# Hiroto1201/Open3D-ML

Measured on AMD Instinct MI355X. Metric: Mpoints/s neighbor-search + sparse-conv fwd; RandLA-Net frames/s, higher is better.
Workload: dtype f32; 1 GPU; C1 fixed_radius_search: layers.FixedRadiusSearch forward (hash build + search) over 64 scenes/GPU x 65,536 U[0,1)^3 pts, r=0.05, L2, int32 idx; scenes_per_gpu=64, parallelism=scene-dp1

## Files before the change

### open3d-ml_amd/csrc/nns_hash.hip

```cpp
#include <algorithm>
#include <cstdlib>

#include "primitives.hpp"
#include "spatial_hash.hpp"

namespace o3dml {

__global__ void __launch_bounds__(256) hash_points_kernel(const float* __restrict__ points, int64_t n, float inv,
                                                          int n_batch, const int64_t* __restrict__ prs,
                                                          const uint32_t* __restrict__ hts,
                                                          uint32_t* __restrict__ bins) {
    __shared__ int64_t s_rs[kLdsSplits];
    __shared__ uint32_t s_tab[kLdsSplits][3];
    const int64_t* rsp = stage_splits(s_rs, prs, n_batch);
    const bool tab = n_batch <= kLdsSplits;
    if (tab) {
        for (int b = threadIdx.x; b < n_batch; b += blockDim.x) {
            const uint32_t first = hts[b], tsize = hts[b + 1] - first;
            s_tab[b][0] = first;
            s_tab[b][1] = tsize;
            s_tab[b][2] = pow64_mod(tsize);
        }
        __syncthreads();
    }
// ... 72 lines not shown
    }
    __syncthreads();
}

__global__ void __launch_bounds__(256) hash_plan_kernel(const int64_t* __restrict__ prs, int nb,
                                                        const uint32_t* __restrict__ hts,
                                                        int64_t* __restrict__ chunk_start,
                                                        int64_t* __restrict__ hist_off, int chunk) {
    hash_plan_block(prs, nb, hts, chunk, chunk_start, hist_off);
}

constexpr int kPlanLds = 512;

__device__ __forceinline__ bool hash_chunk_of(const int64_t* __restrict__ chunk_start, int nb, int& b, int64_t& c) {
    const int64_t w = blockIdx.x;
    if (w >= chunk_start[nb]) return false;
    int lo = 0, hi = nb - 1;
    while (lo < hi) {
        const int mid = (lo + hi + 1) >> 1;
        if (chunk_start[mid] <= w) lo = mid; else hi = mid - 1;
    }
    b = lo;
    c = w - chunk_start[lo];
    return true;
}

template <bool PLAN>
__global__ void __launch_bounds__(256) hash_chunk_hist_kernel(const float* __restrict__ points, float inv, int nb,
                                                              const int64_t* __restrict__ prs,
                                                              const uint32_t* __restrict__ hts,
                                                              int64_t* __restrict__ chunk_start,
                                                              int64_t* __restrict__ hist_off,
                                                              uint32_t* __restrict__ bins, uint32_t* __restrict__ hist,
                                                              int chunk) {
    extern __shared__ uint32_t h[];
    __shared__ int64_t s_plan[PLAN ? 2 * kPlanLds : 1];
    const int64_t* cs = chunk_start;
    const int64_t* ho = hist_off;
    if constexpr (PLAN) {
        hash_plan_block(prs, nb, hts, chunk, s_plan, s_plan + kPlanLds);
        if (blockIdx.x == 0)
            for (int i = threadIdx.x; i <= nb; i += 256) {
                chunk_start[i] = s_plan[i];
                hist_off[i] = s_plan[kPlanLds + i];
            }
        cs = s_plan;
        ho = s_plan + kPlanLds;
    }
    int b;
    int64_t c;
    if (!hash_chunk_of(cs, nb, b, c)) return;
    const int64_t* hist_off_ = ho;
    const uint32_t tsize = hts[b + 1] - hts[b];
    const uint32_t k64 = pow64_mod(tsize);
    for (uint32_t i = threadIdx.x; i < tsize; i += 256) h[i] = 0;
    __syncthreads();
    const int64_t p0 = prs[b] + c * chunk, p1 = min(prs[b + 1], p0 + chunk);
    constexpr int U = 8;
    for (int64_t i0 = p0 + threadIdx.x; i0 < p1; i0 += 256 * U) {
        float px[U], py[U], pz[U];
#pragma unroll
        for (int u = 0; u < U; ++u) {
            const int64_t i = i0 + 256 * u;
            const int64_t j = i < p1 ? i : p0;
            px[u] = points[3 * j];
            py[u] = points[3 * j + 1];
            pz[u] = points[3 * j + 2];
        }
#pragma unroll
        for (int u = 0; u < U; ++u) {
            const int64_t i = i0 + 256 * u;
            if (i < p1) {
                const uint32_t bin = point_bin_k(px[u], py[u], pz[u], inv, tsize, k64);
                bins[i] = bin;
                atomicAdd(&h[bin], 1u);
            }
        }
    }
    __syncthreads();
    uint32_t* out = hist + hist_off_[b] + c * tsize;
    for (uint32_t i = threadIdx.x; i < tsize; i += 256) out[i] = h[i];
}

constexpr int kColBins = 64;
__global__ void __launch_bounds__(256) hash_hist_colscan_kernel(int nslices, const uint32_t* __restrict__ hts,
                                                                const int64_t* __restrict__ chunk_start,
                                                                const int64_t* __restrict__ hist_off,
                                                                uint32_t* __restrict__ hist,
                                                                uint32_t* __restrict__ bin_tot) {
    __shared__ uint32_t qsum[4][kColBins];
    const int b = blockIdx.x / nslices, s = blockIdx.x % nslices;
    const int q = wave_id(), lane = lane_id();
    const uint32_t first = hts[b], tsize = hts[b + 1] - first;
    const uint32_t bin = static_cast<uint32_t>(s * kColBins + lane);
    if (static_cast<uint32_t>(s * kColBins) >= tsize) return;
    const bool valid = bin < tsize;
    const int64_t nchunks = chunk_start[b + 1] - chunk_start[b];
    const int64_t c0 = nchunks * q / 4, c1 = nchunks * (q + 1) / 4;
    uint32_t* H = hist + hist_off[b] + bin;
    uint32_t sum = 0;
    if (valid) {
        int64_t cc = c0;
        for (; cc + 8 <= c1; cc += 8) {
            uint32_t v[8];
#pragma unroll
            for (int u = 0; u < 8; ++u) v[u] = H[(cc + u) * tsize];
            sum += ((v[0] + v[1]) + (v[2] + v[3])) + ((v[4] + v[5]) + (v[6] + v[7]));
        }
        for (; cc < c1; ++cc) sum += H[cc * tsize];
    }
    qsum[q][lane] = sum;
    __syncthreads();
    uint32_t run = 0;
    for (int k = 0; k < q; ++k) run += qsum[k][lane];
    if (valid) {
        if (q == 3) bin_tot[first + bin] = run + sum;
        int64_t cc = c0;
        for (; cc + 8 <= c1; cc += 8) {
            uint32_t v[8];
#pragma unroll
            for (int u = 0; u < 8; ++u) v[u] = H[(cc + u) * tsize];
#pragma unroll
            for (int u = 0; u < 8; ++u) {
                H[(cc + u) * tsize] = run;
                run += v[u];
            }
        }
        for (; cc < c1; ++cc) {
            const uint32_t v = H[cc * tsize];
            H[cc * tsize] = run;
            run += v;
        }
    }
}

template <int CHUNK, int NWV = kHashWaves>
__global__ void __launch_bounds__(NWV * 64) hash_chunk_scatter_kernel(int nb, const int64_t* __restrict__ prs,
                                                                 const uint32_t* __restrict__ hts,
                                                                 const int64_t* __restrict__ chunk_start,
                                                                 const int64_t* __restrict__ hist_off,
                                                                 const uint32_t* __restrict__ bins,
                                                                 const uint32_t* __restrict__ hist,
                                                                 const uint32_t* __restrict__ bin_tot,
                                                                 uint32_t* __restrict__ cell_splits,
                                                                 uint32_t* __restrict__ hti, int max_bins) {
    constexpr int kRows = CHUNK / 64 / NWV;
    extern __shared__ uint32_t wc_all[];
    __shared__ uint32_t wsum[NWV];
    int b;
    int64_t c;
    if (!hash_chunk_of(chunk_start, nb, b, c)) return;
    const int t = threadIdx.x, w = wave_id(), lane = lane_id();
    const uint32_t first = hts[b], tsize = hts[b + 1] - first;
    const int64_t item0 = prs[b], item_end = prs[b + 1];
    const uint32_t* base = hist + hist_off[b] + c * tsize;
    uint32_t* wc = wc_all + w * max_bins;
    uint32_t* bstart = wc_all + NWV * max_bins;
    for (uint32_t i = t; i < tsize; i += NWV * 64)
#pragma unroll
        for (int ww = 0; ww < NWV; ++ww) wc_all[ww * max_bins + i] = 0;
    {
        uint32_t carry = 0;
        for (uint32_t b0 = 0; b0 < tsize; b0 += NWV * 64) {
            const uint32_t i = b0 + t;
            const uint32_t v = i < tsize ? bin_tot[first + i] : 0u;
            const uint32_t inc = wave_inclusive_scan(v);
            if (lane == 63) wsum[w] = inc;
            __syncthreads();
            uint32_t st = carry + inc - v, all = 0;
#pragma unroll
            for (int ww = 0; ww < NWV; ++ww) {
                st += ww < w ? wsum[ww] : 0u;
                all += wsum[ww];
            }
            if (i < tsize) {
                bstart[i] = st;
                if (c == 0) cell_splits[first + i] = static_cast<uint32_t>(item0 + st);
            }
            carry += all;
            __syncthreads();
        }
        if (c == 0 && b == nb - 1 && t == 0) cell_splits[first + tsize] = static_cast<uint32_t>(prs[nb]);
    }
    __syncthreads();
    const int64_t p0 = item0 + c * CHUNK;
    const int64_t pend = min(item_end, p0 + CHUNK);
    const int nbits = tsize > 1 ? 32 - __builtin_clz(tsize - 1) : 0;
    const uint64_t lt = lanemask_lt();
    uint32_t dig[kRows], loff[kRows];
#pragma unroll
    for (int r = 0; r < kRows; ++r) {
        const int64_t i = p0 + (static_cast<int64_t>(w) * kRows + r) * 64 + lane;
        dig[r] = bins[i < pend ? i : p0];
    }
#pragma unroll
    for (int r = 0; r < kRows; ++r) {
        const int64_t i = p0 + (static_cast<int64_t>(w) * kRows + r) * 64 + lane;
        const bool valid = i < pend;
        const uint32_t d = valid ? dig[r] : 0u;
        dig[r] = d;
        uint64_t peers = __builtin_amdgcn_ballot_w64(valid);
        for (int bit = 0; bit < nbits; ++bit) {
            const bool on = (d >> bit) & 1u;
            const uint64_t m = __builtin_amdgcn_ballot_w64(on);
            peers &= on ? m : ~m;
        }
        const uint32_t rank = __popcll(peers & lt);
        const uint32_t before = valid ? wc[d] : 0u;
        loff[r] = before + rank;
        if (valid && rank == 0) wc[d] = before + static_cast<uint32_t>(__popcll(peers));
    }
    __syncthreads();
    for (uint32_t i = t; i < tsize; i += NWV * 64) {
        uint32_t a = bstart[i] + base[i];
#pragma unroll
        for (int ww = 0; ww < NWV; ++ww) {
            const uint32_t cw = wc_all[ww * max_bins + i];
            wc_all[ww * max_bins + i] = a;
            a += cw;
        }
    }
    __syncthreads();
#pragma unroll
    for (int r = 0; r < kRows; ++r) {
        const int64_t i = p0 + (static_cast<int64_t>(w) * kRows + r) * 64 + lane;
        if (i < pend) hti[item0 + wc[dig[r]] + loff[r]] = static_cast<uint32_t>(i);
    }
}

}

using namespace o3dml;

O3DML_API int64_t o3dml_hash_table_splits(int64_t n_batch, const int64_t* points_row_splits_host,
                                          double hash_table_size_factor, int64_t max_hash_table_size,
                                          uint32_t* hash_table_splits_host) {
    hash_table_splits_host[0] = 0;
    for (int64_t b = 0; b < n_batch; ++b) {
        const int64_t nb = points_row_splits_host[b + 1] - points_row_splits_host[b];
        int64_t t = static_cast<int64_t>(hash_table_size_factor * static_cast<double>(nb));
        if (t < 1) t = 1;
        if (t > max_hash_table_size) t = max_hash_table_size;
        hash_table_splits_host[b + 1] = hash_table_splits_host[b] + static_cast<uint32_t>(t);
    }
    return hash_table_splits_host[n_batch];
}

O3DML_API size_t o3dml_build_spatial_hash_table_workspace_size(int64_t n_points, int64_t total_bins) {
    const size_t radix = ws_bytes<uint32_t>(n_points) * 2 + prim::radix_sort_workspace_bytes<uint32_t>(n_points);
    const int64_t nb_ub = total_bins;
    const int64_t hist_ub = 4 * n_points + total_bins;
    const size_t small = ws_bytes<uint32_t>(n_points) + ws_bytes<uint32_t>(hist_ub) +
                         ws_bytes<uint32_t>(total_bins) + 2 * ws_bytes<int64_t>(nb_ub + 1);
    return std::max(radix, small);
}

O3DML_API int o3dml_build_spatial_hash_table(const float* points, int64_t n_points, float radius, int64_t n_batch,
                                             const int64_t* points_row_splits, const uint32_t* hash_table_splits,
                                             const uint32_t* hash_table_splits_host, int64_t total_bins,
                                             uint32_t* hash_table_index, uint32_t* hash_table_cell_splits,
                                             void* workspace, size_t workspace_bytes, void* stream) {
    O3DML_GUARD_BEGIN
    O3DML_REQUIRE(radius > 0.f, "radius must be > 0");
    O3DML_REQUIRE(n_batch >= 1, "need at least one batch item");
    O3DML_REQUIRE(total_bins >= n_batch && total_bins < (int64_t(1) << 32), "invalid hash table size %lld",
                  (long long)total_bins);
    hipStream_t st = as_stream(stream);
    Workspace ws(workspace, workspace_bytes);
    const float inv = 1.0f / (2.0f * radius);
    bool small = hash_table_splits_host != nullptr && n_points > 0;
    uint32_t max_bins = 1;
    for (int64_t b = 0; small && b < n_batch; ++b) {
        const uint32_t tb = hash_table_splits_host[b + 1] - hash_table_splits_host[b];
        max_bins = std::max(max_bins, tb);
        small = tb <= static_cast<uint32_t>(kSmallTable);
    }
    if (small) {
        uint32_t* bins = ws.take<uint32_t>(n_points);
        static const int forced = [] {
            const char* e = std::getenv("O3DML_HASH_CHUNK");
            const int v = e ? std::atoi(e) : 0;
            return (v == 1024 || v == 2048 || v == 4096) ? v : 0;
        }();
        const int chunk = forced ? forced : (ceil_div(n_points, kHashChunk) < 512 ? kHashChunkSmall : kHashChunk);
        uint32_t* hist = ws.take<uint32_t>((kHashChunk / chunk) * n_points + total_bins);
        uint32_t* bin_tot = ws.take<uint32_t>(total_bins);
        int64_t* chunk_start = ws.take<int64_t>(n_batch + 1);
        int64_t* hist_off = ws.take<int64_t>(n_batch + 1);
        const unsigned grid = static_cast<unsigned>(ceil_div(n_points, chunk) + n_batch);
        if (n_batch < kPlanLds) {
            hash_chunk_hist_kernel<true><<<grid, 256, sizeof(uint32_t) * max_bins, st>>>(
                    points, inv, (int)n_batch, points_row_splits, hash_table_splits, chunk_start, hist_off, bins,
                    hist, chunk);
        } else {
            hash_plan_kernel<<<1, 256, 0, st>>>(points_row_splits, (int)n_batch, hash_table_splits, chunk_start,
                                                hist_off, chunk);
            O3DML_LAUNCH_CHECK();
            hash_chunk_hist_kernel<false><<<grid, 256, sizeof(uint32_t) * max_bins, st>>>(
                    points, inv, (int)n_batch, points_row_splits, hash_table_splits, chunk_start, hist_off, bins,
                    hist, chunk);
        }
        O3DML_LAUNCH_CHECK();
        const int nslices = static_cast<int>(ceil_div(max_bins, kColBins));
        hash_hist_colscan_kernel<<<static_cast<unsigned>(n_batch * nslices), 256, 0, st>>>(
                nslices, hash_table_splits, chunk_start, hist_off, hist, bin_tot);
        O3DML_LAUNCH_CHECK();
        const size_t lds = sizeof(uint32_t) * (kHashWaves + 1) * max_bins;
        static const int hw = [] {
            const char* e = std::getenv("O3DML_HASH_WAVES");
            return e ? std::atoi(e) : 4;
        }();
        const size_t lds8 = sizeof(uint32_t) * 9 * max_bins;
        if (chunk == kHashChunkSmall)
            hash_chunk_scatter_kernel<kHashChunkSmall><<<grid, 256, lds, st>>>(
                    (int)n_batch, points_row_splits, hash_table_splits, chunk_start, hist_off, bins, hist, bin_tot,
                    hash_table_cell_splits, hash_table_index, static_cast<int>(max_bins));
        else if (chunk == 2048)
            hash_chunk_scatter_kernel<2048><<<grid, 256, lds, st>>>(
                    (int)n_batch, points_row_splits, hash_table_splits, chunk_start, hist_off, bins, hist, bin_tot,
                    hash_table_cell_splits, hash_table_index, static_cast<int>(max_bins));
        else if (hw == 8 && lds8 <= 65536)
            hash_chunk_scatter_kernel<kHashChunk, 8><<<grid, 512, lds8, st>>>(
                    (int)n_batch, points_row_splits, hash_table_splits, chunk_start, hist_off, bins, hist, bin_tot,
                    hash_table_cell_splits, hash_table_index, static_cast<int>(max_bins));
        else
            hash_chunk_scatter_kernel<kHashChunk><<<grid, 256, lds, st>>>(
                    (int)n_batch, points_row_splits, hash_table_splits, chunk_start, hist_off, bins, hist, bin_tot,
                    hash_table_cell_splits, hash_table_index, static_cast<int>(max_bins));
        O3DML_LAUNCH_CHECK();
        return 0;
    }
    uint32_t* bins = ws.take<uint32_t>(n_points);
    uint32_t* skeys = ws.take<uint32_t>(n_points);
    if (n_points > 0) {
        hash_points_kernel<<<stream_grid(n_points, 256), 256, 0, st>>>(points, n_points, inv, (int)n_batch,
                                                                      points_row_splits, hash_table_splits, bins);
        O3DML_LAUNCH_CHECK();
        prim::radix_sort_pairs<uint32_t>(bins, nullptr, skeys, hash_table_index, n_points,
                                         prim::bits_needed(static_cast<uint64_t>(total_bins - 1)), ws, st);
    }
    bin_boundaries_kernel<<<stream_grid(n_points > 0 ? n_points : total_bins + 1, 256), 256, 0, st>>>(
            skeys, n_points, total_bins, hash_table_cell_splits);
    O3DML_LAUNCH_CHECK();
    O3DML_GUARD_END
}
```

### open3d-ml_amd/csrc/common.hpp

```cpp
#pragma once

#include <hip/hip_runtime.h>

#include <cstdint>
#include <cstdio>
#include <cstring>
#include <string>

#include "../../include/o3dml_amd.h"

#define O3DML_API extern "C" __attribute__((visibility("default")))

namespace o3dml {

void set_error(const char* fmt, ...);
const char* last_error();

struct Error {
    int code;
};

#define O3DML_CHECK_HIP(expr)                                                   \
    do {                                                                        \
        hipError_t _e = (expr);                                                 \
// ... 91 lines not shown
    return (static_cast<size_t>(count < 0 ? 0 : count) * sizeof(T) + 255) & ~size_t(255);
}

__device__ __forceinline__ float sum_slabs(const float* __restrict__ part, int nsplit, int64_t total, int64_t e) {
    float v = 0.f;
    int s = 0;
    for (; s + 16 <= nsplit; s += 16) {
        float t[16];
#pragma unroll
        for (int j = 0; j < 16; ++j) t[j] = part[(s + j) * total + e];
#pragma unroll
        for (int j = 0; j < 16; ++j) v += t[j];
    }
    for (; s < nsplit; ++s) v += part[s * total + e];
    return v;
}

__device__ __forceinline__ int lane_id() { return threadIdx.x & 63; }
__device__ __forceinline__ int wave_id() { return threadIdx.x >> 6; }

__device__ __forceinline__ uint64_t lanemask_lt() {
    const int l = lane_id();
    return l == 0 ? 0ull : (~0ull >> (64 - l));
}

template <class T>
__device__ __forceinline__ T wave_inclusive_scan(T v) {
#pragma unroll
    for (int d = 1; d < 64; d <<= 1) {
        T t = __shfl_up(v, d, 64);
        if (lane_id() >= d) v += t;
    }
    return v;
}

template <class T>
__device__ __forceinline__ T wave_sum(T v) {
#pragma unroll
    for (int d = 32; d >= 1; d >>= 1) v += __shfl_xor(v, d, 64);
    return v;
}

template <class T>
__device__ __forceinline__ T wave_max(T v) {
#pragma unroll
    for (int d = 32; d >= 1; d >>= 1) {
        const T o = __shfl_xor(v, d, 64);
        v = o > v ? o : v;
    }
    return v;
}

__device__ __forceinline__ float dist_l2(float px, float py, float pz, float qx, float qy, float qz) {
    const float dx = px - qx, dy = py - qy, dz = pz - qz;
    return __builtin_fmaf(dz, dz, __builtin_fmaf(dy, dy, dx * dx));
}

enum Metric { kL1 = 0, kL2 = 1, kLinf = 2 };

template <int METRIC>
__device__ __forceinline__ float dist_metric(float px, float py, float pz, float qx, float qy, float qz) {
    if constexpr (METRIC == kL2) {
        return dist_l2(px, py, pz, qx, qy, qz);
    } else {
        const float ax = fabsf(px - qx), ay = fabsf(py - qy), az = fabsf(pz - qz);
        if constexpr (METRIC == kL1) {
            return (ax + ay) + az;
        } else {
            const float m = ax > ay ? ax : ay;
            return m > az ? m : az;
        }
    }
}

__device__ __forceinline__ int batch_of(int64_t i, const int64_t* __restrict__ splits, int n_batch) {
    int lo = 0, hi = n_batch - 1;
    while (lo < hi) {
        int mid = (lo + hi + 1) >> 1;
        if (splits[mid] <= i) lo = mid; else hi = mid - 1;
    }
    return lo;
}

template <int LANE>
__device__ __forceinline__ int write_lane(int v, int x) {
    asm volatile("v_writelane_b32 %0, %1, %2" : "+v"(v) : "s"(x), "i"(LANE));
    return v;
}

constexpr int kBufferFlags = 0x00020000;

constexpr int kLdsSplits = 1024;
__device__ __forceinline__ const int64_t* stage_splits(int64_t* lds, const int64_t* __restrict__ splits,
                                                       int n_batch) {
    if (n_batch + 1 > kLdsSplits) return splits;
    for (int i = threadIdx.x; i <= n_batch; i += blockDim.x) lds[i] = splits[i];
    __syncthreads();
    return lds;
}

__device__ __forceinline__ int64_t xcd_block() {
    const int64_t g = gridDim.x, b = blockIdx.x;
    return (g & 7) ? b : (b & 7) * (g >> 3) + (b >> 3);
}

inline unsigned xcd_grid(int64_t n, int block) {
    int64_t g = ceil_div(n, 4 * static_cast<int64_t>(block));
    g = ((g + 7) / 8) * 8;
    if (g < 8) g = 8;
    if (g > 2048) g = 2048;
    return static_cast<unsigned>(g);
}

}
```

### open3d-ml_amd/csrc/nns_frs.hip

```cpp
#include <algorithm>
#include <cstdlib>
#include <mutex>

#include "primitives.hpp"
#include "spatial_hash.hpp"

namespace o3dml {

__global__ void __launch_bounds__(256) gather_sorted_points_kernel(const float* __restrict__ points,
                                                                   const uint32_t* __restrict__ index, int64_t n,
                                                                   float4* __restrict__ out, int sentinel,
                                                                   int64_t* __restrict__ zero_a, int n_zero_a,
                                                                   int64_t* __restrict__ zero_b) {
    const int64_t per = ceil_div(n, static_cast<int64_t>(gridDim.x));
    const int64_t blk = xcd_block();
    const int64_t e = min(n, (blk + 1) * per);
    constexpr int U = 4;
    for (int64_t j0 = blk * per + threadIdx.x; j0 < e; j0 += U * static_cast<int64_t>(blockDim.x)) {
        uint32_t id[U];
#pragma unroll
        for (int u = 0; u < U; ++u) {
            const int64_t j = j0 + u * static_cast<int64_t>(blockDim.x);
            id[u] = j < e ? index[j] : 0u;
        }
// ... 80 lines not shown
O3DML_DPP_STEP(dmax_rm, "v_max_f32", "row_mirror")
#undef O3DML_DPP_STEP
template <bool MAX>
__device__ __forceinline__ float row_ext_f(float v) {
#if O3DML_FRS_DPPMIN
    if constexpr (MAX) return dmax_rm(dmax_hm(dmax_q2(dmax_q1(v))));
    return dmin_rm(dmin_hm(dmin_q2(dmin_q1(v))));
#else
    auto op = [](float a, float b) { return MAX ? fmaxf(a, b) : fminf(a, b); };
    v = op(v, dpp_f<0xB1>(v));
    v = op(v, dpp_f<0x4E>(v));
    v = op(v, dpp_f<0x141>(v));
    v = op(v, dpp_f<0x140>(v));
    return v;
#endif
}
__device__ __forceinline__ float rdlane_f(float v, int l) {
    return __int_as_float(__builtin_amdgcn_readlane(__float_as_int(v), l));
}
__device__ __forceinline__ float wave_min_f(float v) {
    v = row_ext_f<false>(v);
    return fminf(fminf(rdlane_f(v, 0), rdlane_f(v, 16)), fminf(rdlane_f(v, 32), rdlane_f(v, 48)));
}
__device__ __forceinline__ float wave_max_f(float v) {
    v = row_ext_f<true>(v);
    return fmaxf(fmaxf(rdlane_f(v, 0), rdlane_f(v, 16)), fmaxf(rdlane_f(v, 32), rdlane_f(v, 48)));
}
__device__ __forceinline__ float row0_min_f(float v) { return rdlane_f(row_ext_f<false>(v), 0); }
__device__ __forceinline__ float row0_max_f(float v) { return rdlane_f(row_ext_f<true>(v), 0); }

template <int METRIC>
__device__ __forceinline__ float box_dist(const float4& p, float lx, float ly, float lz, float hx, float hy,
                                          float hz) {
    const float gx = p.x - __builtin_amdgcn_fmed3f(p.x, lx, hx);
    const float gy = p.y - __builtin_amdgcn_fmed3f(p.y, ly, hy);
    const float gz = p.z - __builtin_amdgcn_fmed3f(p.z, lz, hz);
    if constexpr (METRIC == kL2) {
        return __builtin_fmaf(gz, gz, __builtin_fmaf(gy, gy, gx * gx));
    } else if constexpr (METRIC == kL1) {
        return (fabsf(gx) + fabsf(gy)) + fabsf(gz);
    } else {
        const float ax = fabsf(gx), ay = fabsf(gy), az = fabsf(gz);
        const float m = ax > ay ? ax : ay;
        return m > az ? m : az;
    }
}

template <int METRIC>
__device__ __forceinline__ float box_box_dist(float alx, float aly, float alz, float ahx, float ahy, float ahz,
                                              float blx, float bly, float blz, float bhx, float bhy, float bhz) {
    const float gx = fmaxf(fmaxf(alx - bhx, blx - ahx), 0.f);
    const float gy = fmaxf(fmaxf(aly - bhy, bly - ahy), 0.f);
    const float gz = fmaxf(fmaxf(alz - bhz, blz - ahz), 0.f);
    if constexpr (METRIC == kL2) {
        return __builtin_fmaf(gz, gz, __builtin_fmaf(gy, gy, gx * gx));
    } else if constexpr (METRIC == kL1) {
        return (gx + gy) + gz;
    } else {
        const float m = gx > gy ? gx : gy;
        return m > gz ? m : gz;
    }
}

__device__ __forceinline__ int keep_slot(uint64_t km) {
    return static_cast<int>(__builtin_amdgcn_mbcnt_hi(static_cast<uint32_t>(km >> 32),
                                                      __builtin_amdgcn_mbcnt_lo(static_cast<uint32_t>(km), 0u)));
}

__device__ __forceinline__ uint32_t mbcnt64(uint64_t m) {
    return __builtin_amdgcn_mbcnt_hi(static_cast<uint32_t>(m >> 32),
                                     __builtin_amdgcn_mbcnt_lo(static_cast<uint32_t>(m), 0u));
}

__device__ __forceinline__ uint32_t bcnt_add(uint32_t x, uint32_t acc) {
    uint32_t r;
    asm("v_bcnt_u32_b32 %0, %1, %2" : "=v"(r) : "v"(x), "v"(acc));
    return r;
}

__device__ __forceinline__ uint32_t rdlane(int v, uint32_t lane) {
    return static_cast<uint32_t>(__builtin_amdgcn_readlane(v, static_cast<int>(lane)));
}

template <int K>
__device__ __forceinline__ int bin_lanes(int v, const uint32_t* lb) {
    if constexpr (K < 9) return bin_lanes<K + 1>(write_lane<K>(v, static_cast<int>(lb[K])), lb);
    return v;
}

#ifndef O3DML_FRS_NUM_SGPR
#define O3DML_FRS_NUM_SGPR 80
#endif
#ifndef O3DML_FRS_WAVES
#define O3DML_FRS_WAVES 8
#endif
#ifndef O3DML_FRS_ABS16
#define O3DML_FRS_ABS16 1
#endif
#define O3DML_FRS_ATTR \
    __attribute__((amdgpu_num_sgpr(O3DML_FRS_NUM_SGPR), amdgpu_waves_per_eu(DIST ? 1 : O3DML_FRS_WAVES, 8)))
template <int METRIC, bool IGNORE, bool DIST, int MODE, class TIdx, bool REL16>
__global__ void __launch_bounds__(64) O3DML_FRS_ATTR
frs_group_kernel(const float4* __restrict__ pts, uint32_t n_pts, const uint32_t* __restrict__ cs,
                 const float4* __restrict__ qpts, const uint32_t* __restrict__ qsel,
                 const uint32_t* __restrict__ qkeys, int bshift, int64_t m_host, const int64_t* __restrict__ m_dev,
                 float r, float inv, float thr, int nb, const int64_t* __restrict__ qrs,
                 const uint32_t* __restrict__ hts, const int64_t* __restrict__ prs,
                 uint32_t* __restrict__ counts, uint32_t* __restrict__ tidx,
                 float* __restrict__ tdist, uint32_t* __restrict__ over, int64_t* __restrict__ n_over,
                 const int64_t* __restrict__ rs, TIdx* __restrict__ out_idx, float* __restrict__ out_dist,
                 const int64_t* __restrict__ total, int64_t cap, const uint32_t* __restrict__ dir,
                 int64_t dir_cap, int qlog, int64_t dense_w) {
    __shared__ float4 cand[kCandCap];
    __shared__ float4 qsh[64];
    __shared__ int64_t qrow[MODE == 0 ? 1 : 64];
    const int lane = threadIdx.x;
    const float inf = __builtin_huge_valf();
    const float4 far = make_float4(inf, inf, inf, 0.f);
    const int64_t m = MODE == 1 && cap >= 0 && *total > cap ? 0 : (m_dev ? *m_dev : m_host);
    const int64_t nchunks = MODE == 0 ? (m + (1 << qlog) - 1) >> qlog : m;
    const bool pts_rsrc_ok = n_pts < 0x07FFFFFEu;
    const bool sub = dir != nullptr && static_cast<int64_t>(hts[nb]) <= dir_cap;
    const __amdgpu_buffer_rsrc_t rows_rsrc = __builtin_amdgcn_make_buffer_rsrc(
            tidx, static_cast<short>(0), REL16 ? static_cast<int>(m * 2 * kRowCap) : 0, kBufferFlags);
    const __amdgpu_buffer_rsrc_t pts_rsrc = __builtin_amdgcn_make_buffer_rsrc(
            const_cast<float4*>(pts), static_cast<short>(0), static_cast<int>((2u * n_pts + 1u) * 16u), kBufferFlags);
    const int64_t per = (nchunks + 7) >> 3;
    const bool xcd_map = static_cast<int64_t>(gridDim.x) == 8 * per;
    int64_t chunk = xcd_map ? static_cast<int64_t>(blockIdx.x & 7) * per + (blockIdx.x >> 3) : blockIdx.x;
    for (; chunk < nchunks; chunk = xcd_map ? nchunks : chunk + gridDim.x) {
        const int64_t t = MODE == 0 ? (chunk << qlog) + lane : chunk;
        const bool valid = t < m && (MODE == 0 ? lane < (1 << qlog) : lane == 0);
        float4 q4 = far;
        QueryBins qb;
#pragma unroll
        for (int k = 0; k < 9; ++k) qb.b[k] = 0xffffffffu;
        int64_t row = 0;
        uint32_t pbase = 0;
        if (valid) {
            if constexpr (MODE == 0) {
                if (qsel) {
                    const uint32_t qs = qsel[t];
                    if (qpts) {
                        const float* qp = reinterpret_cast<const float*>(qpts) + 3 * static_cast<int64_t>(qs);
                        q4 = make_float4(qp[0], qp[1], qp[2], __uint_as_float(qs));
                    } else {
                        q4 = pts[qs];
                    }
                } else {
                    q4 = qpts[t];
                }
            } else {
                const uint32_t id = over[t];
                const float* qp = reinterpret_cast<const float*>(qpts) + 3 * static_cast<int64_t>(id);
                q4 = make_float4(qp[0], qp[1], qp[2], __uint_as_float(id));
            }
            const uint32_t qid = __float_as_uint(q4.w);
            const int b = qkeys ? (bshift >= 32 ? 0 : static_cast<int>(qkeys[t] >> bshift)) : batch_of(qid, qrs, nb);
            if constexpr (REL16) pbase = static_cast<uint32_t>(prs[b]);
            const uint32_t first = hts[b], tsize = hts[b + 1] - first;
            qb = query_bins(q4.x, q4.y, q4.z, r, inv, first, tsize);
            if constexpr (MODE == 1) row = dense_w > 0 ? static_cast<int64_t>(qid) * dense_w : rs[qid];
        }
        uint64_t todo = __builtin_amdgcn_ballot_w64(valid);
        while (todo) {
            const int leader = __builtin_ctzll(todo);
            uint32_t lb[9];
            bool same = valid;
#pragma unroll
            for (int k = 0; k < 9; ++k) {
                lb[k] = rdlane(static_cast<int>(qb.b[k]), leader);
                same = same && qb.b[k] == lb[k];
            }
            const uint64_t gm = __builtin_amdgcn_ballot_w64(same);
            const uint32_t gbase = REL16 ? rdlane(static_cast<int>(pbase), leader) : 0u;
            todo &= ~gm;
            const int ng = __popcll(gm);
            __syncthreads();
            if (same) {
                const uint32_t slot = mbcnt64(gm);
                qsh[slot] = q4;
                if constexpr (MODE == 1) qrow[slot] = row;
            }
            float lx, ly, lz, hx, hy, hz;
            if (ng <= 16) {
                __syncthreads();
                const float4 v = lane < ng ? qsh[lane & 15] : far;
                const float4 w = lane < ng ? v : make_float4(-inf, -inf, -inf, 0.f);
                lx = row0_min_f(v.x), ly = row0_min_f(v.y), lz = row0_min_f(v.z);
                hx = row0_max_f(w.x), hy = row0_max_f(w.y), hz = row0_max_f(w.z);
            } else {
                lx = wave_min_f(same ? q4.x : inf), ly = wave_min_f(same ? q4.y : inf),
                lz = wave_min_f(same ? q4.z : inf);
                hx = wave_max_f(same ? q4.x : -inf), hy = wave_max_f(same ? q4.y : -inf),
                hz = wave_max_f(same ? q4.z : -inf);
            }
            const uint32_t split = kLaneSplit[ng];
            const int S = static_cast<int>(split & 0xffu);
            const int g = static_cast<int>((static_cast<uint32_t>(lane) * (split >> 8)) >> 16);
            const int sl = lane - g * S;
            __syncthreads();
            float4 mq = far;
            int64_t mrow = 0;
            if (g < ng) {
                mq = qsh[g];
                mrow = MODE == 0 ? static_cast<int64_t>(__float_as_uint(mq.w)) : qrow[g];
            }
            uint32_t cnt = 0;
            const uint32_t row_b = static_cast<uint32_t>(mrow) * (2u * kRowCap);
            const uint64_t gmask = S == 64 ? ~0ull : (g < ng ? ((1ull << S) - 1ull) << (g * S) : 0ull);
            const uint32_t gm_lo = static_cast<uint32_t>(gmask), gm_hi = static_cast<uint32_t>(gmask >> 32);
            uint32_t vst, vlen;
            int nbk;
            {
                const uint32_t vb = static_cast<uint32_t>(bin_lanes<0>(-1, lb));
                uint32_t s0 = 0, e0 = 0;
                uint4 w0 = {}, w1 = {}, w2 = {}, w3 = {}, w4 = {}, w5 = {};
                if (lane < 9) {
                    s0 = cs[vb];
                    e0 = cs[vb + 1];
                    if (sub) {
                        const uint4* dp = reinterpret_cast<const uint4*>(dir + static_cast<size_t>(vb) * kDirWords);
                        w0 = dp[0], w1 = dp[1], w2 = dp[2], w3 = dp[3], w4 = dp[4], w5 = dp[5];
                    }
                }
                const uint32_t prev = static_cast<uint32_t>(
                        __builtin_amdgcn_update_dpp(-1, static_cast<int>(vb), 0x111, 0xF, 0xF, false));
                const bool first = lane < 9 && e0 > s0 && prev != vb;
                uint32_t st = s0, ln = e0 - s0;
                if (first && sub) {
                    const uint32_t n0 = w0.x, n1 = w0.y, n2 = ln - n0 - n1;
                    auto f = [](uint32_t u) { return __uint_as_float(u); };
                    const bool r0 = n0 > 0 && box_box_dist<METRIC>(f(w1.x), f(w1.y), f(w1.z), f(w1.w), f(w2.x),
                                                                   f(w2.y), lx, ly, lz, hx, hy, hz) <= thr;
                    const bool r1 = n1 > 0 && box_box_dist<METRIC>(f(w2.z), f(w2.w), f(w3.x), f(w3.y), f(w3.z),
                                                                   f(w3.w), lx, ly, lz, hx, hy, hz) <= thr;
                    const bool r2 = n2 > 0 && box_box_dist<METRIC>(f(w4.x), f(w4.y), f(w4.z), f(w4.w), f(w5.x),
                                                                   f(w5.y), lx, ly, lz, hx, hy, hz) <= thr;
                    const int nr = static_cast<int>(r0) + static_cast<int>(r1) + static_cast<int>(r2);
                    const uint32_t base = n_pts + 1 + s0;
                    if (nr == 0) {
                        ln = 0;
                    } else if (nr == 1) {
                        st = r0 && n0 == ln ? s0 : base + (r0 ? 0u : (r1 ? n0 : n0 + n1));
                        ln = r0 ? n0 : (r1 ? n1 : n2);
                    }
                }
                const bool live = first && ln > 0;
                const uint64_t km = __builtin_amdgcn_ballot_w64(live);
                nbk = __popcll(km);
                uint32_t* tab = reinterpret_cast<uint32_t*>(cand);
                if (live) {
                    const uint32_t j = mbcnt64(km);
                    tab[j] = st;
                    tab[16 + j] = ln;
                }
                __syncthreads();
                vst = lane < nbk ? tab[lane] : 0u;
                vlen = lane < nbk ? tab[16 + lane] : 0u;
                __syncthreads();
            }
#if O3DML_DIAG == 2
            nbk = 0;
#endif
            const int fill_lim = kCandCap - 64 * kStreamU - (S - 1);
            int bk = 0;
            uint32_t boff = 0;
            auto round_src = [&]() -> uint32_t {
                if (bk >= nbk) return n_pts;
                const uint32_t st0 = rdlane(static_cast<int>(vst), bk) + boff;
                const uint32_t t = rdlane(static_cast<int>(vlen), bk) - boff;
                if (t > 64) {
                    boff += 64;
                    return st0 + lane;
                }
                const uint32_t n1 = rdlane(static_cast<int>(vlen), bk + 1);
                const uint32_t d1 = rdlane(static_cast<int>(vst), bk + 1) - t;
                const uint32_t src = static_cast<uint32_t>(lane) < t ? st0 + lane : d1 + lane;
                if (t + n1 <= 64) {
                    bk += 2;
                    boff = 0;
                } else {
                    bk += 1;
                    boff = 64 - t;
                }
                return static_cast<uint32_t>(lane) < t + n1 ? src : n_pts;
            };
            auto load_step = [&](float4* c, auto buf) {
                uint32_t src[kStreamU];
#pragma unroll
                for (int u = 0; u < kStreamU; ++u) src[u] = round_src();
                if constexpr (decltype(buf)::value) {
#pragma unroll
                    for (int u = 0; u < kStreamU; ++u)
                        c[u] = __builtin_bit_cast(float4,
                                                  __builtin_amdgcn_raw_buffer_load_b128(pts_rsrc, src[u] * 16u, 0, 0));
                } else {
#pragma unroll
                    for (int u = 0; u < kStreamU; ++u) c[u] = pts[src[u]];
                }
            };
            auto stream_and_test = [&](auto buf) {
            int nc = 0;
            while (true) {
#if O3DML_FRS_DMA
                if constexpr (decltype(buf)::value) {
                    while (bk < nbk && nc <= fill_lim) {
                        uint32_t src[kStreamU];
#pragma unroll
                        for (int u = 0; u < kStreamU; ++u) src[u] = round_src();
                        const int nc0 = nc;
#pragma unroll
                        for (int u = 0; u < kStreamU; ++u)
                            __builtin_amdgcn_raw_ptr_buffer_load_lds(pts_rsrc, (frs_lds_ptr)(cand + nc0 + 64 * u), 16,
                                                                     src[u] * 16u, 0, 0, 0);
                        asm volatile("s_waitcnt vmcnt(0)" ::: "memory");
#pragma unroll
                        for (int u = 0; u < kStreamU; ++u) {
                            float4 c = cand[nc0 + 64 * u + lane];
                            const bool keep = box_dist<METRIC>(c, lx, ly, lz, hx, hy, hz) <= thr;
                            const uint64_t km = __builtin_amdgcn_ballot_w64(keep);
                            if constexpr (REL16 && !O3DML_FRS_ABS16) c.w = __uint_as_float(__float_as_uint(c.w) - gbase);
                            if (keep)
                                (cand + nc)[keep_slot(km)] = c;
                            nc += __popcll(km);
                        }
                    }
                }
                while (!decltype(buf)::value && bk < nbk && nc <= fill_lim) {
#else
                while (bk < nbk && nc <= fill_lim) {
#endif
                    float4 c[kStreamU];
                    load_step(c, buf);
#pragma unroll
                    for (int u = 0; u < kStreamU; ++u) {
                        const bool keep = box_dist<METRIC>(c[u], lx, ly, lz, hx, hy, hz) <= thr;
                        const uint64_t km = __builtin_amdgcn_ballot_w64(keep);
                        if constexpr (REL16 && !O3DML_FRS_ABS16)
                            c[u].w = __uint_as_float(__float_as_uint(c[u].w) - gbase);
                        if (keep)
                            (cand + nc)[keep_slot(km)] = c[u];
                        nc += __popcll(km);
                    }
                }
                const int ncp = static_cast<int>(((static_cast<uint32_t>(nc + S - 1) * (split >> 8)) >> 16) *
                                                 static_cast<uint32_t>(S));
                if (nc + lane < ncp) cand[nc + lane] = far;
                __syncthreads();
// ... 967 lines not shown
```

Measured before the change: 4033 Mpoints/s.

## Fold histogram column scan into scatter kernel, dropping separate colscan pass

```diff
diff --git a/open3d-ml_amd/csrc/nns_hash.hip b/open3d-ml_amd/csrc/nns_hash.hip
--- a/open3d-ml_amd/csrc/nns_hash.hip
+++ b/open3d-ml_amd/csrc/nns_hash.hip
@@ -178,58 +178,6 @@
     for (uint32_t i = threadIdx.x; i < tsize; i += 256) out[i] = h[i];
 }
 
-constexpr int kColBins = 64;
-__global__ void __launch_bounds__(256) hash_hist_colscan_kernel(int nslices, const uint32_t* __restrict__ hts,
-                                                                const int64_t* __restrict__ chunk_start,
-                                                                const int64_t* __restrict__ hist_off,
-                                                                uint32_t* __restrict__ hist,
-                                                                uint32_t* __restrict__ bin_tot) {
-    __shared__ uint32_t qsum[4][kColBins];
-    const int b = blockIdx.x / nslices, s = blockIdx.x % nslices;
-    const int q = wave_id(), lane = lane_id();
-    const uint32_t first = hts[b], tsize = hts[b + 1] - first;
-    const uint32_t bin = static_cast<uint32_t>(s * kColBins + lane);
-    if (static_cast<uint32_t>(s * kColBins) >= tsize) return;
-    const bool valid = bin < tsize;
-    const int64_t nchunks = chunk_start[b + 1] - chunk_start[b];
-    const int64_t c0 = nchunks * q / 4, c1 = nchunks * (q + 1) / 4;
-    uint32_t* H = hist + hist_off[b] + bin;
-    uint32_t sum = 0;
-    if (valid) {
-        int64_t cc = c0;
-        for (; cc + 8 <= c1; cc += 8) {
-            uint32_t v[8];
-#pragma unroll
-            for (int u = 0; u < 8; ++u) v[u] = H[(cc + u) * tsize];
-            sum += ((v[0] + v[1]) + (v[2] + v[3])) + ((v[4] + v[5]) + (v[6] + v[7]));
-        }
-        for (; cc < c1; ++cc) sum += H[cc * tsize];
-    }
-    qsum[q][lane] = sum;
-    __syncthreads();
-    uint32_t run = 0;
-    for (int k = 0; k < q; ++k) run += qsum[k][lane];
-    if (valid) {
-        if (q == 3) bin_tot[first + bin] = run + sum;
-        int64_t cc = c0;
-        for (; cc + 8 <= c1; cc += 8) {
-            uint32_t v[8];
-#pragma unroll
-            for (int u = 0; u < 8; ++u) v[u] = H[(cc + u) * tsize];
-#pragma unroll
-            for (int u = 0; u < 8; ++u) {
-                H[(cc + u) * tsize] = run;
-                run += v[u];
-            }
-        }
-        for (; cc < c1; ++cc) {
-            const uint32_t v = H[cc * tsize];
-            H[cc * tsize] = run;
-            run += v;
-        }
-    }
-}
-
 template <int CHUNK, int NWV = kHashWaves>
 __global__ void __launch_bounds__(NWV * 64) hash_chunk_scatter_kernel(int nb, const int64_t* __restrict__ prs,
                                                                  const uint32_t* __restrict__ hts,
@@ -237,7 +185,6 @@
                                                                  const int64_t* __restrict__ hist_off,
                                                                  const uint32_t* __restrict__ bins,
                                                                  const uint32_t* __restrict__ hist,
-                                                                 const uint32_t* __restrict__ bin_tot,
                                                                  uint32_t* __restrict__ cell_splits,
                                                                  uint32_t* __restrict__ hti, int max_bins) {
     constexpr int kRows = CHUNK / 64 / NWV;
@@ -249,7 +196,9 @@
     const int t = threadIdx.x, w = wave_id(), lane = lane_id();
     const uint32_t first = hts[b], tsize = hts[b + 1] - first;
     const int64_t item0 = prs[b], item_end = prs[b + 1];
-    const uint32_t* base = hist + hist_off[b] + c * tsize;
+    const uint32_t* H = hist + hist_off[b];
+    const int nchunks = static_cast<int>(chunk_start[b + 1] - chunk_start[b]);
+    const int ci = static_cast<int>(c);
     uint32_t* wc = wc_all + w * max_bins;
     uint32_t* bstart = wc_all + NWV * max_bins;
     for (uint32_t i = t; i < tsize; i += NWV * 64)
@@ -259,7 +208,26 @@
         uint32_t carry = 0;
         for (uint32_t b0 = 0; b0 < tsize; b0 += NWV * 64) {
             const uint32_t i = b0 + t;
-            const uint32_t v = i < tsize ? bin_tot[first + i] : 0u;
+            uint32_t v = 0, pre = 0;
+            if (i < tsize) {
+                const uint32_t* col = H + i;
+                int cc = 0;
+                for (; cc + 16 <= nchunks; cc += 16) {
+                    uint32_t x[16];
+#pragma unroll
+                    for (int u = 0; u < 16; ++u) x[u] = col[static_cast<int64_t>(cc + u) * tsize];
+#pragma unroll
+                    for (int u = 0; u < 16; ++u) {
+                        v += x[u];
+                        pre += cc + u < ci ? x[u] : 0u;
+                    }
+                }
+                for (; cc < nchunks; ++cc) {
+                    const uint32_t x = col[static_cast<int64_t>(cc) * tsize];
+                    v += x;
+                    pre += cc < ci ? x : 0u;
+                }
+            }
             const uint32_t inc = wave_inclusive_scan(v);
             if (lane == 63) wsum[w] = inc;
             __syncthreads();
@@ -270,7 +238,7 @@
                 all += wsum[ww];
             }
             if (i < tsize) {
-                bstart[i] = st;
+                bstart[i] = st + pre;
                 if (c == 0) cell_splits[first + i] = static_cast<uint32_t>(item0 + st);
             }
             carry += all;
@@ -308,7 +276,7 @@
     }
     __syncthreads();
     for (uint32_t i = t; i < tsize; i += NWV * 64) {
-        uint32_t a = bstart[i] + base[i];
+        uint32_t a = bstart[i];
 #pragma unroll
         for (int ww = 0; ww < NWV; ++ww) {
             const uint32_t cw = wc_all[ww * max_bins + i];
@@ -346,8 +314,7 @@
     const size_t radix = ws_bytes<uint32_t>(n_points) * 2 + prim::radix_sort_workspace_bytes<uint32_t>(n_points);
     const int64_t nb_ub = total_bins;
     const int64_t hist_ub = 4 * n_points + total_bins;
-    const size_t small = ws_bytes<uint32_t>(n_points) + ws_bytes<uint32_t>(hist_ub) +
-                         ws_bytes<uint32_t>(total_bins) + 2 * ws_bytes<int64_t>(nb_ub + 1);
+    const size_t small = ws_bytes<uint32_t>(n_points) + ws_bytes<uint32_t>(hist_ub) + 2 * ws_bytes<int64_t>(nb_ub + 1);
     return std::max(radix, small);
 }
 
@@ -378,9 +345,10 @@
             const int v = e ? std::atoi(e) : 0;
             return (v == 1024 || v == 2048 || v == 4096) ? v : 0;
         }();
-        const int chunk = forced ? forced : (ceil_div(n_points, kHashChunk) < 512 ? kHashChunkSmall : kHashChunk);
+        const bool few = ceil_div(n_points, kHashChunk) < 512 &&
+                         ceil_div(n_points, kHashChunkSmall) * static_cast<int64_t>(max_bins) <= 64 * 1024;
+        const int chunk = forced ? forced : (few ? kHashChunkSmall : kHashChunk);
         uint32_t* hist = ws.take<uint32_t>((kHashChunk / chunk) * n_points + total_bins);
-        uint32_t* bin_tot = ws.take<uint32_t>(total_bins);
         int64_t* chunk_start = ws.take<int64_t>(n_batch + 1);
         int64_t* hist_off = ws.take<int64_t>(n_batch + 1);
         const unsigned grid = static_cast<unsigned>(ceil_div(n_points, chunk) + n_batch);
@@ -397,31 +365,18 @@
                     hist, chunk);
         }
         O3DML_LAUNCH_CHECK();
-        const int nslices = static_cast<int>(ceil_div(max_bins, kColBins));
-        hash_hist_colscan_kernel<<<static_cast<unsigned>(n_batch * nslices), 256, 0, st>>>(
-                nslices, hash_table_splits, chunk_start, hist_off, hist, bin_tot);
-        O3DML_LAUNCH_CHECK();
         const size_t lds = sizeof(uint32_t) * (kHashWaves + 1) * max_bins;
-        static const int hw = [] {
-            const char* e = std::getenv("O3DML_HASH_WAVES");
-            return e ? std::atoi(e) : 4;
-        }();
-        const size_t lds8 = sizeof(uint32_t) * 9 * max_bins;
         if (chunk == kHashChunkSmall)
             hash_chunk_scatter_kernel<kHashChunkSmall><<<grid, 256, lds, st>>>(
-                    (int)n_batch, points_row_splits, hash_table_splits, chunk_start, hist_off, bins, hist, bin_tot,
+                    (int)n_batch, points_row_splits, hash_table_splits, chunk_start, hist_off, bins, hist,
                     hash_table_cell_splits, hash_table_index, static_cast<int>(max_bins));
         else if (chunk == 2048)
             hash_chunk_scatter_kernel<2048><<<grid, 256, lds, st>>>(
-                    (int)n_batch, points_row_splits, hash_table_splits, chunk_start, hist_off, bins, hist, bin_tot,
-                    hash_table_cell_splits, hash_table_index, static_cast<int>(max_bins));
-        else if (hw == 8 && lds8 <= 65536)
-            hash_chunk_scatter_kernel<kHashChunk, 8><<<grid, 512, lds8, st>>>(
-                    (int)n_batch, points_row_splits, hash_table_splits, chunk_start, hist_off, bins, hist, bin_tot,
+                    (int)n_batch, points_row_splits, hash_table_splits, chunk_start, hist_off, bins, hist,
                     hash_table_cell_splits, hash_table_index, static_cast<int>(max_bins));
         else
             hash_chunk_scatter_kernel<kHashChunk><<<grid, 256, lds, st>>>(
-                    (int)n_batch, points_row_splits, hash_table_splits, chunk_start, hist_off, bins, hist, bin_tot,
+                    (int)n_batch, points_row_splits, hash_table_splits, chunk_start, hist_off, bins, hist,
                     hash_table_cell_splits, hash_table_index, static_cast<int>(max_bins));
         O3DML_LAUNCH_CHECK();
         return 0;
```

Measured after the change: 4049 Mpoints/s, median of 6. No clear change (+0.4%).

## Batch bin-table setup for up to seven query groups per wave pass

Applied to the files above, without the earlier changes.

```diff
diff --git a/open3d-ml_amd/csrc/common.hpp b/open3d-ml_amd/csrc/common.hpp
--- a/open3d-ml_amd/csrc/common.hpp
+++ b/open3d-ml_amd/csrc/common.hpp
@@ -197,12 +197,6 @@
     return lo;
 }
 
-template <int LANE>
-__device__ __forceinline__ int write_lane(int v, int x) {
-    asm volatile("v_writelane_b32 %0, %1, %2" : "+v"(v) : "s"(x), "i"(LANE));
-    return v;
-}
-
 constexpr int kBufferFlags = 0x00020000;
 
 constexpr int kLdsSplits = 1024;
diff --git a/open3d-ml_amd/csrc/nns_frs.hip b/open3d-ml_amd/csrc/nns_frs.hip
--- a/open3d-ml_amd/csrc/nns_frs.hip
+++ b/open3d-ml_amd/csrc/nns_frs.hip
@@ -186,10 +186,12 @@
     return static_cast<uint32_t>(__builtin_amdgcn_readlane(v, static_cast<int>(lane)));
 }
 
-template <int K>
-__device__ __forceinline__ int bin_lanes(int v, const uint32_t* lb) {
-    if constexpr (K < 9) return bin_lanes<K + 1>(write_lane<K>(v, static_cast<int>(lb[K])), lb);
-    return v;
+__device__ __forceinline__ int32_t float_key(float f) {
+    const int32_t i = __float_as_int(f);
+    return i ^ ((i >> 31) & 0x7fffffff);
+}
+__device__ __forceinline__ uint32_t key_float(int32_t k) {
+    return static_cast<uint32_t>(k ^ ((k >> 31) & 0x7fffffff));
 }
 
 #ifndef O3DML_FRS_NUM_SGPR
@@ -267,74 +269,85 @@
             if constexpr (MODE == 1) row = dense_w > 0 ? static_cast<int64_t>(qid) * dense_w : rs[qid];
         }
         uint64_t todo = __builtin_amdgcn_ballot_w64(valid);
+        int ngrp = 0;
+        uint32_t goff = 0;
+        uint32_t mytag = 0;
+        int vgrp = 0;
         while (todo) {
             const int leader = __builtin_ctzll(todo);
-            uint32_t lb[9];
             bool same = valid;
 #pragma unroll
-            for (int k = 0; k < 9; ++k) {
-                lb[k] = rdlane(static_cast<int>(qb.b[k]), leader);
-                same = same && qb.b[k] == lb[k];
-            }
+            for (int k = 0; k < 9; ++k) same = same && qb.b[k] == rdlane(static_cast<int>(qb.b[k]), leader);
             const uint64_t gm = __builtin_amdgcn_ballot_w64(same);
-            const uint32_t gbase = REL16 ? rdlane(static_cast<int>(pbase), leader) : 0u;
             todo &= ~gm;
-            const int ng = __popcll(gm);
-            __syncthreads();
+            const uint32_t ng = static_cast<uint32_t>(__popcll(gm));
             if (same) {
                 const uint32_t slot = mbcnt64(gm);
-                qsh[slot] = q4;
-                if constexpr (MODE == 1) qrow[slot] = row;
+                mytag = static_cast<uint32_t>(ngrp) | (slot == 0 ? 0x300u : 0x200u) | ((goff + slot) << 16);
             }
-            float lx, ly, lz, hx, hy, hz;
-            if (ng <= 16) {
+            if (lane == ngrp) vgrp = static_cast<int>(ng | (goff << 8) | (static_cast<uint32_t>(leader) << 16));
+            goff += ng;
+            ++ngrp;
+        }
+        uint32_t* const tab = reinterpret_cast<uint32_t*>(cand);
+        __syncthreads();
+        if (valid) {
+            qsh[mytag >> 16] = q4;
+            if constexpr (MODE == 1) qrow[mytag >> 16] = row;
+        }
+        uint32_t vst = 0, vlen = 0;
+        uint64_t km = 0;
+        int gi = 0, nbat = 0;
+        for (int grp = 0; grp < ngrp; ++grp, ++gi) {
+            if (gi == nbat) {
+                uint2* const seg = reinterpret_cast<uint2*>(cand) + 64;
+                int bl = lane;
+                uint32_t kmax = INT32_MAX, kmin = static_cast<uint32_t>(INT32_MIN), zero = 0u;
+                asm volatile("" : "+v"(bl), "+v"(kmax), "+v"(kmin), "+v"(zero));
+                const int tg = (bl * 57) >> 9, tk = bl - 9 * tg;
                 __syncthreads();
-                const float4 v = lane < ng ? qsh[lane & 15] : far;
-                const float4 w = lane < ng ? v : make_float4(-inf, -inf, -inf, 0.f);
-                lx = row0_min_f(v.x), ly = row0_min_f(v.y), lz = row0_min_f(v.z);
-                hx = row0_max_f(w.x), hy = row0_max_f(w.y), hz = row0_max_f(w.z);
-            } else {
-                lx = wave_min_f(same ? q4.x : inf), ly = wave_min_f(same ? q4.y : inf),
-                lz = wave_min_f(same ? q4.z : inf);
-                hx = wave_max_f(same ? q4.x : -inf), hy = wave_max_f(same ? q4.y : -inf),
-                hz = wave_max_f(same ? q4.z : -inf);
-            }
-            const uint32_t split = kLaneSplit[ng];
-            const int S = static_cast<int>(split & 0xffu);
-            const int g = static_cast<int>((static_cast<uint32_t>(lane) * (split >> 8)) >> 16);
-            const int sl = lane - g * S;
-            __syncthreads();
-            float4 mq = far;
-            int64_t mrow = 0;
-            if (g < ng) {
-                mq = qsh[g];
-                mrow = MODE == 0 ? static_cast<int64_t>(__float_as_uint(mq.w)) : qrow[g];
-            }
-            uint32_t cnt = 0;
-            const uint32_t row_b = static_cast<uint32_t>(mrow) * (2u * kRowCap);
-            const uint64_t gmask = S == 64 ? ~0ull : (g < ng ? ((1ull << S) - 1ull) << (g * S) : 0ull);
-            const uint32_t gm_lo = static_cast<uint32_t>(gmask), gm_hi = static_cast<uint32_t>(gmask >> 32);
-            uint32_t vst, vlen;
-            int nbk;
-            {
-                const uint32_t vb = static_cast<uint32_t>(bin_lanes<0>(-1, lb));
-                uint32_t s0 = 0, e0 = 0;
+                const uint32_t rel = (mytag & 0xffu) - static_cast<uint32_t>(grp);
+                if ((mytag & 0x100u) != 0u && rel < 7u) {
+                    uint4* const tp = reinterpret_cast<uint4*>(tab) + 4 * rel;
+                    tp[0] = make_uint4(kmax, kmax, kmax, kmin);
+                    tp[1] = make_uint4(kmin, kmin, qb.b[0], qb.b[1]);
+                    tp[2] = make_uint4(qb.b[2], qb.b[3], qb.b[4], qb.b[5]);
+                    tp[3] = make_uint4(qb.b[6], qb.b[7], qb.b[8], zero);
+                }
+                seg[bl] = make_uint2(zero, zero);
+                __syncthreads();
+                if ((mytag & 0x200u) != 0u && rel < 7u) {
+                    const float4 me = qsh[mytag >> 16];
+                    int32_t* const k = reinterpret_cast<int32_t*>(tab) + 16 * rel;
+                    const int32_t kx = float_key(me.x), ky = float_key(me.y), kz = float_key(me.z);
+                    __hip_atomic_fetch_min(k + 0, kx, __ATOMIC_RELAXED, __HIP_MEMORY_SCOPE_WORKGROUP);
+                    __hip_atomic_fetch_min(k + 1, ky, __ATOMIC_RELAXED, __HIP_MEMORY_SCOPE_WORKGROUP);
+                    __hip_atomic_fetch_min(k + 2, kz, __ATOMIC_RELAXED, __HIP_MEMORY_SCOPE_WORKGROUP);
+                    __hip_atomic_fetch_max(k + 3, kx, __ATOMIC_RELAXED, __HIP_MEMORY_SCOPE_WORKGROUP);
+                    __hip_atomic_fetch_max(k + 4, ky, __ATOMIC_RELAXED, __HIP_MEMORY_SCOPE_WORKGROUP);
+                    __hip_atomic_fetch_max(k + 5, kz, __ATOMIC_RELAXED, __HIP_MEMORY_SCOPE_WORKGROUP);
+                }
+                __syncthreads();
+                const bool task_ok = tg < 7 && grp + tg < ngrp;
+                const uint32_t* const tq = tab + 16 * tg;
+                const uint32_t vb = tab[task_ok ? 16 * tg + 6 + tk : 6];
+                const uint32_t prev = tq[5 + tk];
+                const uint4 b0 = reinterpret_cast<const uint4*>(tq)[0];
+                const uint2 b1 = reinterpret_cast<const uint2*>(tq)[2];
+                const uint32_t s0 = cs[vb], e0 = cs[vb + 1];
                 uint4 w0 = {}, w1 = {}, w2 = {}, w3 = {}, w4 = {}, w5 = {};
-                if (lane < 9) {
-                    s0 = cs[vb];
-                    e0 = cs[vb + 1];
-                    if (sub) {
-                        const uint4* dp = reinterpret_cast<const uint4*>(dir + static_cast<size_t>(vb) * kDirWords);
-                        w0 = dp[0], w1 = dp[1], w2 = dp[2], w3 = dp[3], w4 = dp[4], w5 = dp[5];
-                    }
-                }
-                const uint32_t prev = static_cast<uint32_t>(
-                        __builtin_amdgcn_update_dpp(-1, static_cast<int>(vb), 0x111, 0xF, 0xF, false));
-                const bool first = lane < 9 && e0 > s0 && prev != vb;
+                if (sub) {
+                    const uint4* dp = reinterpret_cast<const uint4*>(dir + static_cast<size_t>(vb) * kDirWords);
+                    w0 = dp[0], w1 = dp[1], w2 = dp[2], w3 = dp[3], w4 = dp[4], w5 = dp[5];
+                }
+                const bool first = task_ok && e0 > s0 && (tk == 0 || prev != vb);
                 uint32_t st = s0, ln = e0 - s0;
                 if (first && sub) {
+                    auto f = [](uint32_t u) { return __uint_as_float(u); };
+                    auto kf = [](uint32_t k) { return __uint_as_float(key_float(static_cast<int32_t>(k))); };
+                    const float lx = kf(b0.x), ly = kf(b0.y), lz = kf(b0.z), hx = kf(b0.w), hy = kf(b1.x),
+                                hz = kf(b1.y);
                     const uint32_t n0 = w0.x, n1 = w0.y, n2 = ln - n0 - n1;
-                    auto f = [](uint32_t u) { return __uint_as_float(u); };
                     const bool r0 = n0 > 0 && box_box_dist<METRIC>(f(w1.x), f(w1.y), f(w1.z), f(w1.w), f(w2.x),
                                                                    f(w2.y), lx, ly, lz, hx, hy, hz) <= thr;
                     const bool r1 = n1 > 0 && box_box_dist<METRIC>(f(w2.z), f(w2.w), f(w3.x), f(w3.y), f(w3.z),
@@ -351,24 +364,51 @@
                     }
                 }
                 const bool live = first && ln > 0;
-                const uint64_t km = __builtin_amdgcn_ballot_w64(live);
-                nbk = __popcll(km);
-                uint32_t* tab = reinterpret_cast<uint32_t*>(cand);
-                if (live) {
-                    const uint32_t j = mbcnt64(km);
-                    tab[j] = st;
-                    tab[16 + j] = ln;
-                }
+                km = __builtin_amdgcn_ballot_w64(live);
+                nbat = __popcll(km) > 57 ? 6 : min(7, ngrp - grp);
+                if (live && tg < nbat) seg[mbcnt64(km) + tg] = make_uint2(st, ln);
                 __syncthreads();
-                vst = lane < nbk ? tab[lane] : 0u;
-                vlen = lane < nbk ? tab[16 + lane] : 0u;
+                const uint2 sg = seg[bl];
+                vst = sg.x, vlen = sg.y;
                 __syncthreads();
+                gi = 0;
             }
+            const uint32_t ginfo = rdlane(vgrp, static_cast<uint32_t>(grp));
+            const int ng = static_cast<int>(ginfo & 0xffu);
+            const uint32_t gslot = (ginfo >> 8) & 0xffu, leader = ginfo >> 16;
+            const uint32_t gbase = REL16 ? rdlane(static_cast<int>(pbase), leader) : 0u;
+            float lx, ly, lz, hx, hy, hz;
+            if (ng <= 16) {
+                const float4 v = lane < ng ? qsh[gslot + (lane & 15)] : far;
+                const float4 w = lane < ng ? v : make_float4(-inf, -inf, -inf, 0.f);
+                lx = row0_min_f(v.x), ly = row0_min_f(v.y), lz = row0_min_f(v.z);
+                hx = row0_max_f(w.x), hy = row0_max_f(w.y), hz = row0_max_f(w.z);
+            } else {
+                const float4 v = lane < ng ? qsh[gslot + lane] : far;
+                const float4 w = lane < ng ? v : make_float4(-inf, -inf, -inf, 0.f);
+                lx = wave_min_f(v.x), ly = wave_min_f(v.y), lz = wave_min_f(v.z);
+                hx = wave_max_f(w.x), hy = wave_max_f(w.y), hz = wave_max_f(w.z);
+            }
+            const uint32_t split = kLaneSplit[ng];
+            const int S = static_cast<int>(split & 0xffu);
+            const int g = static_cast<int>((static_cast<uint32_t>(lane) * (split >> 8)) >> 16);
+            const int sl = lane - g * S;
+            float4 mq = far;
+            int64_t mrow = 0;
+            if (g < ng) {
+                mq = qsh[gslot + g];
+                mrow = MODE == 0 ? static_cast<int64_t>(__float_as_uint(mq.w)) : qrow[gslot + g];
+            }
+            uint32_t cnt = 0;
+            const uint32_t row_b = static_cast<uint32_t>(mrow) * (2u * kRowCap);
+            const uint64_t gmask = S == 64 ? ~0ull : (g < ng ? ((1ull << S) - 1ull) << (g * S) : 0ull);
+            const uint32_t gm_lo = static_cast<uint32_t>(gmask), gm_hi = static_cast<uint32_t>(gmask >> 32);
+            int bk = __popcll(km & ((1ull << (9 * gi)) - 1ull)) + gi;
+            int nbk = bk + __popcll((km >> (9 * gi)) & 0x1ffull);
 #if O3DML_DIAG == 2
-            nbk = 0;
+            nbk = bk;
 #endif
             const int fill_lim = kCandCap - 64 * kStreamU - (S - 1);
-            int bk = 0;
             uint32_t boff = 0;
             auto round_src = [&]() -> uint32_t {
                 if (bk >= nbk) return n_pts;
```

Measured after the change: 4006 Mpoints/s before, 4158 Mpoints/s after (median of 6 runs). +3.8%, better.
